# Project-Arda/bgls

Hardware: AMD Instinct MI355X
Metric: aggregate-verify signer-pairs/sec (higher is better)
Workload: dtype u32; 1 GPU; altbn128 VerifyAggregateSignature, one 1048576-signer batch, keys+msgs resident in HBM; curve=altbn128, signers=1048576, signers_per_gpu=1048576, in_flight=8

## Files before the change

bgls_amd/csrc/fp.hpp:

```cpp
#pragma once
#include <stdint.h>
#include "constants_gen.hpp"

#if defined(__HIPCC__)
#include <hip/hip_runtime.h>
#define BGLS_HD __host__ __device__ __forceinline__
#define BGLS_FN __host__ __device__ __noinline__
#else
#define BGLS_HD inline __attribute__((always_inline))
#define BGLS_FN __attribute__((noinline))
#endif

namespace bgls {

typedef uint32_t u32;
typedef uint64_t u64;
typedef int32_t i32;
typedef int64_t i64;

BGLS_HD u32 addc(u32 a, u32 b, u32& c) {
  u32 co;
  u32 r = __builtin_addc(a, b, c, &co);
  c = co;
  return r;
// ... 393 lines not shown
BGLS_FN Fp<C> fp_inv_ds(const Fp<C>& a) {
  constexpr int L = C::L;
  constexpr int NW = (32 * L + 29) / 30 + ((32 * L) % 30 == 0 ? 1 : 0);
  constexpr i32 M30 = (i32)((1u << 30) - 1u);
  static_assert(30 * NW >= 32 * L + 2, "limbs hold (-2p, 2p)");
  auto limb = [](const u32* w, int i) -> i32 {
    const int bit = 30 * i, q = bit >> 5, sh = bit & 31;
    if (q >= L) return 0;
    u64 x = w[q];
    if (q + 1 < L) x |= (u64)w[q + 1] << 32;
    return (i32)((u32)(x >> sh) & (u32)M30);
  };
  i32 f[NW], g[NW], d[NW], e[NW], m[NW];
#pragma unroll
  for (int i = 0; i < NW; ++i) {
    m[i] = limb(C::P, i);
    f[i] = m[i];
    g[i] = limb(a.v, i);
    d[i] = 0;
    e[i] = i == 0 ? 1 : 0;
  }
  u32 minv = C::P[0];
  minv *= 2u - C::P[0] * minv;
  minv *= 2u - C::P[0] * minv;
  minv *= 2u - C::P[0] * minv;
  minv *= 2u - C::P[0] * minv;
  minv *= 2u - C::P[0] * minv;
  i32 zeta = -1;
  for (int batch = 0; batch < 64; ++batch) {
    i32 u = 1, v = 0, q = 0, r = 1;
    {
      u32 fl = (u32)f[0] | ((u32)f[1] << 30), gl = (u32)g[0] | ((u32)g[1] << 30);
#pragma unroll
      for (int i = 0; i < 30; ++i) {
        i32 c1 = zeta >> 31;
        const i32 c2 = -(i32)(gl & 1u);
        const u32 x = (fl ^ (u32)c1) - (u32)c1;
        const i32 y = (u ^ c1) - c1, z = (v ^ c1) - c1;
        gl += x & (u32)c2;
        q += y & c2;
        r += z & c2;
        c1 &= c2;
        zeta = (zeta ^ c1) - 1;
        fl += gl & (u32)c1;
        u += q & c1;
        v += r & c1;
        gl >>= 1;
        u = (i32)((u32)u << 1);
        v = (i32)((u32)v << 1);
      }
    }
    {
      const i32 sd = d[NW - 1] >> 31, se = e[NW - 1] >> 31;
      i32 md = (u & sd) + (v & se), me = (q & sd) + (r & se);
      i64 cd = (i64)u * d[0] + (i64)v * e[0], ce = (i64)q * d[0] + (i64)r * e[0];
      md -= (i32)((minv * (u32)cd + (u32)md) & (u32)M30);
      me -= (i32)((minv * (u32)ce + (u32)me) & (u32)M30);
      cd += (i64)m[0] * md;
      ce += (i64)m[0] * me;
      cd >>= 30;
      ce >>= 30;
#pragma unroll
      for (int i = 1; i < NW; ++i) {
        cd += (i64)u * d[i] + (i64)v * e[i] + (i64)m[i] * md;
        ce += (i64)q * d[i] + (i64)r * e[i] + (i64)m[i] * me;
        d[i - 1] = (i32)cd & M30;
        e[i - 1] = (i32)ce & M30;
        cd >>= 30;
        ce >>= 30;
      }
      d[NW - 1] = (i32)cd;
      e[NW - 1] = (i32)ce;
    }
    u32 gnz;
    {
      i64 cf = (i64)u * f[0] + (i64)v * g[0], cg = (i64)q * f[0] + (i64)r * g[0];
      cf >>= 30;
      cg >>= 30;
      gnz = 0;
#pragma unroll
      for (int i = 1; i < NW; ++i) {
        cf += (i64)u * f[i] + (i64)v * g[i];
        cg += (i64)q * f[i] + (i64)r * g[i];
        f[i - 1] = (i32)cf & M30;
        g[i - 1] = (i32)cg & M30;
        gnz |= (u32)g[i - 1];
        cf >>= 30;
        cg >>= 30;
      }
      f[NW - 1] = (i32)cf;
      g[NW - 1] = (i32)cg;
      gnz |= (u32)g[NW - 1];
    }
#if defined(__HIP_DEVICE_COMPILE__)
    if (__ballot(gnz != 0) == 0ull) break;
#else
    if (gnz == 0) break;
#endif
  }
  u32 fone = (u32)f[0] ^ 1u, fmone = (u32)(f[0] ^ M30);
#pragma unroll
  for (int i = 1; i < NW; ++i) { fone |= (u32)f[i]; fmone |= (u32)(f[i] ^ (i == NW - 1 ? -1 : M30)); }
  if (fone != 0 && fmone != 0) return fp_zero<C>();
  const i32 sf = fone == 0 ? 0 : -1;
  i64 c = 0;
  u32 w[L + 1];
  {
    u64 acc = 0;
    int have = 0, wi = 0;
    i64 carry = 0;
#pragma unroll
    for (int i = 0; i < NW; ++i) {
      carry += (i64)((d[i] ^ sf) - sf) + 2 * (i64)m[i];
      const u32 lo = (u32)carry & (u32)M30;
      carry >>= 30;
      acc |= (u64)lo << have;
      have += 30;
      if (have >= 32) {
        if (wi <= L) w[wi] = (u32)acc;
        ++wi;
        acc >>= 32;
        have -= 32;
      }
    }
    acc |= (u64)(u32)carry << have;
    while (wi <= L) { w[wi++] = (u32)acc; acc >>= 32; }
    (void)c;
  }
  Fp<C> rr;
#pragma unroll
  for (int j = 0; j < L; ++j) rr.v[j] = w[j];
  u32 top = w[L];
#pragma unroll
  for (int k = 0; k < 4; ++k) {
    u32 bw = 0;
    u32 t[L];
#pragma unroll
    for (int j = 0; j < L; ++j) t[j] = subb(rr.v[j], C::P[j], bw);
    const bool ge = top != 0 || bw == 0;
    if (ge) {
#pragma unroll
      for (int j = 0; j < L; ++j) rr.v[j] = t[j];
      top -= bw;
    }
  }
  const Fp<C> r2 = fp_load<C>(C::R2);
  return fp_mul_inl<C>(fp_mul_inl<C>(rr, r2), r2);
}
template <class C>
BGLS_HD Fp<C> fp_inv(const Fp<C>& a) {
  return fp_inv_ds<C>(a);
}

template <int L, int LC>
BGLS_HD void fp_jacobi_phase(u32 (&a)[L], u32 (&n)[L], u32& t, bool& done) {
  for (int guard = 0; guard < 64 * L + 64; ++guard) {
    if (!done) {
      const u32 low = a[0];
      const u32 sft = low ? (u32)__builtin_ctz(low) : 31u;
#pragma unroll
      for (int j = 0; j < LC - 1; ++j) a[j] = (u32)((((u64)a[j + 1] << 32) | a[j]) >> sft);
      a[LC - 1] >>= sft;
      const u32 n8 = n[0] & 7u;
      t ^= (sft & 1u) & (u32)(n8 == 3u || n8 == 5u);
      const bool odd = (a[0] & 1u) != 0;
      u32 d[LC], e[LC];
      u32 bw = 0, bw2 = 0;
#pragma unroll
      for (int j = 0; j < LC; ++j) d[j] = subb(a[j], n[j], bw);
#pragma unroll
      for (int j = 0; j < LC; ++j) e[j] = subb(n[j], a[j], bw2);
      const bool lt = bw != 0;
      const bool swp = odd && lt;
      t ^= (u32)(swp && (a[0] & 3u) == 3u && (n[0] & 3u) == 3u);
      u32 z = 0;
#pragma unroll
      for (int j = 0; j < LC; ++j) {
        const u32 na = odd ? (lt ? e[j] : d[j]) : a[j];
        n[j] = swp ? a[j] : n[j];
        a[j] = na;
        z |= na;
      }
      if (z == 0) done = true;
    }
    bool again = !done, shrink = false;
    if constexpr (LC > 2) shrink = !done && ((a[LC - 1] | a[LC - 2] | n[LC - 1] | n[LC - 2]) != 0);
#if defined(__HIP_DEVICE_COMPILE__)
    again = __ballot(again) != 0;
    if constexpr (LC > 2) shrink = __ballot(shrink) != 0;
#endif
    if (!again) return;
    if constexpr (LC > 2) {
      if (!shrink) return;
    }
  }
}
template <int L, int LC>
BGLS_HD void fp_jacobi_phases(u32 (&a)[L], u32 (&n)[L], u32& t, bool& done) {
  fp_jacobi_phase<L, LC>(a, n, t, done);
  if constexpr (LC > 2) fp_jacobi_phases<L, LC - 2>(a, n, t, done);
}
template <class C>
BGLS_FN int fp_jacobi(const Fp<C>& x) {
  constexpr int L = C::L;
  static_assert(L % 2 == 0, "limb pairs");
  u32 a[L], n[L];
  u32 nz = 0;
#pragma unroll
  for (int j = 0; j < L; ++j) {
    a[j] = x.v[j];
    n[j] = C::P[j];
    nz |= a[j];
  }
  u32 t = 0;
  bool done = nz == 0;
  fp_jacobi_phases<L, L>(a, n, t, done);
  if (nz == 0) return 0;
  u32 one = n[0] ^ 1u;
#pragma unroll
  for (int j = 1; j < L; ++j) one |= n[j];
  if (one != 0) return 0;
  return t ? -1 : 1;
}

template <class C>
BGLS_HD Fp<C> fp_sqrt_candidate(const Fp<C>& a) {
  return fp_pow_w4<C, C::L>(a, C::EXP_SQRT);
}

template <class C>
BGLS_HD Fp<C> fp_from_be(const uint8_t* b) {
  Fp<C> r;
#pragma unroll
  for (int j = 0; j < C::L; ++j) {
    const uint8_t* q = b + 4 * (C::L - 1 - j);
    r.v[j] = ((u32)q[0] << 24) | ((u32)q[1] << 16) | ((u32)q[2] << 8) | (u32)q[3];
  }
  return r;
}

template <class C>
BGLS_HD void fp_to_be(uint8_t* b, const Fp<C>& a) {
#pragma unroll
  for (int j = 0; j < C::L; ++j) {
    uint8_t* q = b + 4 * (C::L - 1 - j);
    q[0] = (uint8_t)(a.v[j] >> 24);
    q[1] = (uint8_t)(a.v[j] >> 16);
    q[2] = (uint8_t)(a.v[j] >> 8);
    q[3] = (uint8_t)(a.v[j]);
  }
}

}
```

bgls_amd/csrc/h2c.hpp:

```cpp
#pragma once
#include "curve.hpp"
#include "hashes.hpp"

namespace bgls {

inline BGLS_FN bool bn_h2c_try(const uint8_t* msg, size_t len, u32 counter, Fp<BN254>& x, Fp<BN254>& r) {
  typedef BN254 C;
  ByteSrc src;
  src.msg = msg;
  src.len = len;
  src.pre[0] = (uint8_t)counter;
  src.npre = 1;
  src.nsuf = 0;
  u32 d[8];
  keccak256_legacy(src, d);
  Fp<C> h;
#pragma unroll
  for (int j = 0; j < 8; ++j) h.v[j] = d[7 - j];
  x = fp_to_mont<C>(h);
  Fp<C> y2 = fp_add<C>(fp_mul<C>(fp_sqr<C>(x), x), fp_load<C>(C::B));
  r = fp_sqrt_candidate<C>(y2);
  return fp_eq<C>(fp_sqr<C>(r), y2);
}

inline BGLS_FN bool bn_h2c_test(const uint8_t* msg, size_t len, u32 counter, Fp<BN254>& x, Fp<BN254>& y2) {
  typedef BN254 C;
  ByteSrc src;
  src.msg = msg;
  src.len = len;
  src.pre[0] = (uint8_t)counter;
  src.npre = 1;
  src.nsuf = 0;
  u32 d[8];
  keccak256_legacy(src, d);
  Fp<C> h;
#pragma unroll
  for (int j = 0; j < 8; ++j) h.v[j] = d[7 - j];
  x = fp_to_mont<C>(h);
  y2 = fp_add<C>(fp_mul<C>(fp_sqr<C>(x), x), fp_load<C>(C::B));
  return fp_jacobi<C>(y2) >= 0;
}

inline BGLS_FN u32 bn_h2c_sign(const uint8_t* msg, size_t len) {
  ByteSrc src;
  src.msg = msg;
  src.len = len;
  src.pre[0] = 0xFF;
  src.npre = 1;
  src.nsuf = 0;
  u32 d[8];
  keccak256_legacy(src, d);
  return d[7] & 1u;
}

inline BGLS_FN bool bn_hash_to_g1(const uint8_t* msg, size_t len, Aff<F1<BN254>>& out) {
  typedef BN254 C;
  for (u32 c = 0; c < 256; ++c) {
    Fp<C> x, r;
    if (bn_h2c_try(msg, len, c, x, r)) {
      if (bn_h2c_sign(msg, len)) r = fp_neg<C>(r);
      out.x = x;
      out.y = r;
      out.inf = false;
      return true;
    }
  }
  return false;
}

template <class C>
BGLS_HD bool fp_plain_parity(const Fp<C>& a) {
  Fp<C> d;
  u32 bw = 0;
#pragma unroll
  for (int j = 0; j < C::L; ++j) d.v[j] = subb(C::P[j], a.v[j], bw);
  u32 b2 = 0;
#pragma unroll
  for (int j = 0; j < C::L; ++j) (void)subb(d.v[j], a.v[j], b2);
  return b2 != 0;
}

inline BGLS_FN void bls_h2c_digest(const uint8_t* msg, size_t len, int k, u32 (&d)[16]) {
  ByteSrc src;
  src.msg = msg;
  src.len = len;
  src.npre = 0;
  src.pre[0] = 0;
  src.suf[0] = 'G';
  src.suf[1] = '1';
  src.suf[2] = '_';
  src.suf[3] = (uint8_t)('0' + k);
  src.nsuf = 4;
  blake2b512(src, d);
}
inline BGLS_FN Fp<BLS381> bls_h2c_t(const uint8_t* msg, size_t len, int k, Fp<BLS381>& t_mont) {
  typedef BLS381 C;
  u32 d[16];
  bls_h2c_digest(msg, len, k, d);
  Fp<C> lo, hi = fp_zero<C>();
#pragma unroll
  for (int j = 0; j < 12; ++j) lo.v[j] = d[15 - j];
#pragma unroll
  for (int j = 0; j < 4; ++j) hi.v[j] = d[3 - j];
  t_mont = fp_add<C>(fp_mul<C>(lo, fp_load<C>(C::R2)), fp_mul<C>(hi, fp_load<C>(C::R3)));
  return fp_from_mont<C>(t_mont);
}

inline BGLS_FN Aff<F1<BLS381>> bls_sw_encode(const Fp<BLS381>& t_mont, bool t_parity) {
  typedef BLS381 C;
  const Fp<C> one = fp_one<C>();
  const Fp<C> b = fp_load<C>(C::B);
  Fp<C> t2 = fp_sqr<C>(t_mont);
  Fp<C> u = fp_add<C>(fp_add<C>(t2, one), b);
  Fp<C> v = fp_mul3<C>(t2);
  Fp<C> I = fp_inv<C>(fp_mul<C>(u, v));
  Fp<C> inv_u = fp_mul<C>(I, v);
  Fp<C> w = fp_mul<C>(fp_mul<C>(fp_load<C>(C::SQRT_M3), t_mont), inv_u);
  Fp<C> x = fp_sub<C>(fp_load<C>(C::Z_SW), fp_mul<C>(t_mont, w));
  Fp<C> y;
  bool found = false;
  for (int i = 0; i < 3 && !found; ++i) {
    if (i == 1) x = fp_sub<C>(fp_neg<C>(x), one);
    if (i == 2) x = fp_sub<C>(one, fp_mul<C>(fp_mul<C>(fp_sqr<C>(u), u), I));
    Fp<C> g = fp_add<C>(fp_mul<C>(fp_sqr<C>(x), x), b);
    y = fp_sqrt_candidate<C>(g);
    found = (i == 2) || fp_eq<C>(fp_sqr<C>(y), g);
  }
  if (fp_plain_parity<C>(fp_from_mont<C>(y)) != t_parity) y = fp_neg<C>(y);
  return {x, y, false};
}

enum : u32 { H2C_INF = 0, H2C_PLUS_G1 = 1, H2C_MINUS_G1 = 2, H2C_SW = 3, H2C_PENDING = 4 };

struct BlsSwPrep {
  Fp<BLS381> x0, x2;
};
inline BGLS_FN BlsSwPrep bls_sw_prep(const Fp<BLS381>& t_mont) {
  typedef BLS381 C;
  const Fp<C> one = fp_one<C>();
  Fp<C> t2 = fp_sqr<C>(t_mont);
  Fp<C> u = fp_add<C>(fp_add<C>(t2, one), fp_load<C>(C::B));
  Fp<C> v = fp_mul3<C>(t2);
  Fp<C> I = fp_inv<C>(fp_mul<C>(u, v));
  Fp<C> w = fp_mul<C>(fp_mul<C>(fp_load<C>(C::SQRT_M3), t_mont), fp_mul<C>(I, v));
  BlsSwPrep r;
  r.x0 = fp_sub<C>(fp_load<C>(C::Z_SW), fp_mul<C>(t_mont, w));
  r.x2 = fp_sub<C>(one, fp_mul<C>(fp_mul<C>(fp_sqr<C>(u), u), I));
  return r;
}
inline BGLS_FN bool bls_sw_try(const Fp<BLS381>& x, Fp<BLS381>& y) {
  typedef BLS381 C;
  Fp<C> g = fp_add<C>(fp_mul<C>(fp_sqr<C>(x), x), fp_load<C>(C::B));
  y = fp_sqrt_candidate<C>(g);
  return fp_eq<C>(fp_sqr<C>(y), g);
}

template <class F>
BGLS_FN Jac<F> jac_mul_jac(const Jac<F>& p, const u32* k, int nbits) {
  Jac<F> r = jac_inf<F>();
  for (int i = nbits - 1; i >= 0; --i) {
    r = jac_dbl<F>(r);
    if ((k[i >> 5] >> (i & 31)) & 1u) r = jac_add<F>(r, p);
  }
  return r;
}

inline BGLS_FN Jac<F1<BLS381>> bls_hash_to_g1_jac(const uint8_t* msg, size_t len) {
  typedef BLS381 C;
  typedef F1<C> F;
  Jac<F> sw_sum = jac_inf<F>();
  Jac<F> special = jac_inf<F>();
  const Aff<F> g1 = {fp_load<C>(C::G1X), fp_load<C>(C::G1Y), false};
  for (int k = 0; k < 2; ++k) {
    Fp<C> tm;
    Fp<C> t = bls_h2c_t(msg, len, k, tm);
    if (fp_is_zero<C>(t)) continue;
    if (fp_eq<C>(t, fp_load<C>(C::FT_ROOT1))) {
      special = jac_add_aff<F>(special, g1);
    } else if (fp_eq<C>(t, fp_load<C>(C::FT_ROOT2))) {
      special = jac_add_aff<F>(special, aff_neg<F>(g1));
    } else {
      sw_sum = jac_add_aff<F>(sw_sum, bls_sw_encode(tm, fp_plain_parity<C>(t)));
    }
  }
  Jac<F> r = jac_mul_jac<F>(sw_sum, C::COFACTOR, C::COFACTOR_BITS);
  return jac_add<F>(r, special);
}

inline BGLS_FN Aff<F1<BLS381>> bls_hash_to_g1(const uint8_t* msg, size_t len) {
  return jac_to_aff<F1<BLS381>>(bls_hash_to_g1_jac(msg, len));
}

}
```

bgls_amd/csrc/hashes.hpp:

```cpp
#pragma once
#include "fp.hpp"

namespace bgls {

struct ByteSrc {
  const uint8_t* msg;
  size_t len;
  uint8_t pre[1];
  int npre;
  uint8_t suf[4];
  int nsuf;
  BGLS_HD size_t total() const { return (size_t)npre + len + (size_t)nsuf; }
  BGLS_HD u32 at(size_t pos) const {
    if (pos < (size_t)npre) return pre[0];
    pos -= npre;
    if (pos < len) return msg[pos];
    pos -= len;
    return suf[pos & 3];
  }
  BGLS_HD u64 le64(size_t pos, size_t total) const {
    if (pos >= (size_t)npre && pos + 8 <= (size_t)npre + len) {
      u64 w;
      __builtin_memcpy(&w, msg + (pos - (size_t)npre), 8);
      return w;
    }
    u64 w = 0;
#pragma unroll
    for (int b = 0; b < 8; ++b) {
      const size_t q = pos + b;
      const u32 byte = q < total ? at(q) : 0u;
      w |= (u64)byte << (8 * b);
    }
    return w;
  }
};

BGLS_HD u64 rotl64(u64 x, int n) { return (x << n) | (x >> (64 - n)); }
BGLS_HD u64 rotr64(u64 x, int n) { return (x >> n) | (x << (64 - n)); }

#if defined(__HIP_DEVICE_COMPILE__)
#define BGLS_TABLE __device__ __constant__ const
#else
#define BGLS_TABLE static const
#endif

BGLS_TABLE u64 KECCAK_RC[24] = {
    0x0000000000000001ull, 0x0000000000008082ull, 0x800000000000808Aull, 0x8000000080008000ull,
    0x000000000000808Bull, 0x0000000080000001ull, 0x8000000080008081ull, 0x8000000000008009ull,
    0x000000000000008Aull, 0x0000000000000088ull, 0x0000000080008009ull, 0x000000008000000Aull,
    0x000000008000808Bull, 0x800000000000008Bull, 0x8000000000008089ull, 0x8000000000008003ull,
    0x8000000000008002ull, 0x8000000000000080ull, 0x000000000000800Aull, 0x800000008000000Aull,
    0x8000000080008081ull, 0x8000000000008080ull, 0x0000000080000001ull, 0x8000000080008008ull};

BGLS_HD void keccak_f1600(u64 (&st)[25]) {
  constexpr int rotc[24] = {1, 3, 6, 10, 15, 21, 28, 36, 45, 55, 2, 14, 27, 41, 56, 8, 25, 43, 62, 18, 39, 61, 20, 44};
  constexpr int piln[24] = {10, 7, 11, 17, 18, 3, 5, 16, 8, 21, 24, 4, 15, 23, 19, 13, 12, 2, 20, 14, 22, 9, 6, 1};
  for (int round = 0; round < 24; ++round) {
    u64 bc[5];
#pragma unroll
    for (int i = 0; i < 5; ++i) bc[i] = st[i] ^ st[i + 5] ^ st[i + 10] ^ st[i + 15] ^ st[i + 20];
#pragma unroll
    for (int i = 0; i < 5; ++i) {
      u64 t = bc[(i + 4) % 5] ^ rotl64(bc[(i + 1) % 5], 1);
#pragma unroll
      for (int j = 0; j < 25; j += 5) st[j + i] ^= t;
    }
    u64 t = st[1];
#pragma unroll
    for (int i = 0; i < 24; ++i) {
      int j = piln[i];
      u64 b0 = st[j];
      st[j] = rotl64(t, rotc[i]);
      t = b0;
    }
#pragma unroll
    for (int j = 0; j < 25; j += 5) {
#pragma unroll
      for (int i = 0; i < 5; ++i) bc[i] = st[j + i];
#pragma unroll
      for (int i = 0; i < 5; ++i) st[j + i] ^= (~bc[(i + 1) % 5]) & bc[(i + 2) % 5];
    }
    st[0] ^= KECCAK_RC[round];
  }
}

inline BGLS_FN void keccak256_legacy(const ByteSrc& src, u32 (&out_be)[8]) {
  constexpr size_t RATE = 136;
  u64 st[25];
#pragma unroll
  for (int i = 0; i < 25; ++i) st[i] = 0;
  const size_t total = src.total();
  const size_t nblk = total / RATE + 1;
  for (size_t blk = 0; blk < nblk; ++blk) {
    const bool last = (blk + 1 == nblk);
#pragma unroll
    for (int i = 0; i < 17; ++i) {
      const size_t pos = blk * RATE + 8 * i;
      u64 w = src.le64(pos, total);
      if (total >= pos && total < pos + 8) w |= (u64)0x01u << (8 * (total - pos));
      if (last && i == 16) w ^= (u64)0x80u << 56;
      st[i] ^= w;
    }
    keccak_f1600(st);
  }
#pragma unroll
  for (int i = 0; i < 4; ++i) {
    u32 lo = (u32)st[i], hi = (u32)(st[i] >> 32);
    out_be[2 * i] = __builtin_bswap32(lo);
    out_be[2 * i + 1] = __builtin_bswap32(hi);
  }
}

BGLS_TABLE u64 BLAKE2B_IV[8] = {0x6a09e667f3bcc908ull, 0xbb67ae8584caa73bull, 0x3c6ef372fe94f82bull,
                                0xa54ff53a5f1d36f1ull, 0x510e527fade682d1ull, 0x9b05688c2b3e6c1full,
                                0x1f83d9abfb41bd6bull, 0x5be0cd19137e2179ull};
BGLS_TABLE uint8_t BLAKE2B_SIGMA[12][16] = {
    {0, 1, 2, 3, 4, 5, 6, 7, 8, 9, 10, 11, 12, 13, 14, 15}, {14, 10, 4, 8, 9, 15, 13, 6, 1, 12, 0, 2, 11, 7, 5, 3},
    {11, 8, 12, 0, 5, 2, 15, 13, 10, 14, 3, 6, 7, 1, 9, 4}, {7, 9, 3, 1, 13, 12, 11, 14, 2, 6, 5, 10, 4, 0, 15, 8},
    {9, 0, 5, 7, 2, 4, 10, 15, 14, 1, 11, 12, 6, 8, 3, 13}, {2, 12, 6, 10, 0, 11, 8, 3, 4, 13, 7, 5, 15, 14, 1, 9},
    {12, 5, 1, 15, 14, 13, 4, 10, 0, 7, 6, 3, 9, 2, 8, 11}, {13, 11, 7, 14, 12, 1, 3, 9, 5, 0, 15, 4, 8, 6, 2, 10},
    {6, 15, 14, 9, 11, 3, 0, 8, 12, 2, 13, 7, 1, 4, 10, 5}, {10, 2, 8, 4, 7, 6, 1, 5, 15, 11, 9, 14, 3, 12, 13, 0},
    {0, 1, 2, 3, 4, 5, 6, 7, 8, 9, 10, 11, 12, 13, 14, 15}, {14, 10, 4, 8, 9, 15, 13, 6, 1, 12, 0, 2, 11, 7, 5, 3}};

BGLS_HD void blake2b_g(u64 (&v)[16], int a, int b, int c, int d, u64 x, u64 y) {
  v[a] = v[a] + v[b] + x;
  v[d] = rotr64(v[d] ^ v[a], 32);
  v[c] = v[c] + v[d];
  v[b] = rotr64(v[b] ^ v[c], 24);
  v[a] = v[a] + v[b] + y;
  v[d] = rotr64(v[d] ^ v[a], 16);
  v[c] = v[c] + v[d];
  v[b] = rotr64(v[b] ^ v[c], 63);
}

BGLS_HD void blake2b_compress(u64 (&h)[8], const u64 (&m)[16], u64 t, bool last) {
  u64 v[16];
#pragma unroll
  for (int i = 0; i < 8; ++i) {
    v[i] = h[i];
    v[i + 8] = BLAKE2B_IV[i];
  }
  v[12] ^= t;
  if (last) v[14] = ~v[14];
  for (int r = 0; r < 12; ++r) {
    const uint8_t* s = BLAKE2B_SIGMA[r];
    blake2b_g(v, 0, 4, 8, 12, m[s[0]], m[s[1]]);
    blake2b_g(v, 1, 5, 9, 13, m[s[2]], m[s[3]]);
    blake2b_g(v, 2, 6, 10, 14, m[s[4]], m[s[5]]);
    blake2b_g(v, 3, 7, 11, 15, m[s[6]], m[s[7]]);
    blake2b_g(v, 0, 5, 10, 15, m[s[8]], m[s[9]]);
    blake2b_g(v, 1, 6, 11, 12, m[s[10]], m[s[11]]);
    blake2b_g(v, 2, 7, 8, 13, m[s[12]], m[s[13]]);
    blake2b_g(v, 3, 4, 9, 14, m[s[14]], m[s[15]]);
  }
#pragma unroll
  for (int i = 0; i < 8; ++i) h[i] ^= v[i] ^ v[i + 8];
}

inline BGLS_FN void blake2b512(const ByteSrc& src, u32 (&out_be)[16]) {
  u64 h[8];
#pragma unroll
  for (int i = 0; i < 8; ++i) h[i] = BLAKE2B_IV[i];
  h[0] ^= 0x01010040ull;
  const size_t total = src.total();
  const size_t nblk = total == 0 ? 1 : (total + 127) / 128;
  for (size_t blk = 0; blk < nblk; ++blk) {
    u64 m[16];
    for (int i = 0; i < 16; ++i) m[i] = src.le64(blk * 128 + 8 * (size_t)i, total);
    const bool last = (blk + 1 == nblk);
    blake2b_compress(h, m, last ? (u64)total : (u64)(blk + 1) * 128, last);
  }
#pragma unroll
  for (int i = 0; i < 8; ++i) {
    u32 lo = (u32)h[i], hi = (u32)(h[i] >> 32);
    out_be[2 * i] = __builtin_bswap32(lo);
    out_be[2 * i + 1] = __builtin_bswap32(hi);
  }
}

BGLS_HD void blake2xb_root_init(u64 (&h)[8], u32 xof_len) {
#pragma unroll
  for (int i = 0; i < 8; ++i) h[i] = BLAKE2B_IV[i];
  h[0] ^= 0x01010040ull;
  h[1] ^= (u64)xof_len << 32;
}
inline BGLS_FN void blake2xb_node(const u64 (&root)[8], u32 i, u32 xof_len, u32 take, u64 (&out)[8]) {
#pragma unroll
  for (int k = 0; k < 8; ++k) out[k] = BLAKE2B_IV[k];
  out[0] ^= (u64)take | (64ull << 32);
  out[1] ^= (u64)i | ((u64)xof_len << 32);
  out[2] ^= 64ull << 8;
  u64 m[16];
#pragma unroll
  for (int k = 0; k < 8; ++k) {
    m[k] = root[k];
    m[k + 8] = 0;
  }
  blake2b_compress(out, m, 64, true);
}

}
```

bgls_amd/csrc/k_hash.hip:

```cpp
#include <stdlib.h>
#include "dev_common.hpp"
#include "h2c.hpp"
#include "launch.hpp"
#include "rx_pow.hpp"
#include "rx_jac1.hpp"
#include "h2c_x.hpp"

using namespace bgls;

__device__ __forceinline__ uint64_t msg_hash64(const uint8_t* p, size_t n, uint64_t seed) {
  uint64_t h = 0xcbf29ce484222325ull ^ seed;
  for (size_t i = 0; i < n; ++i) {
    h ^= p[i];
    h *= 0x100000001b3ull;
  }
  h ^= h >> 29;
  h *= 0xbf58476d1ce4e5b9ull;
  h ^= h >> 32;
  return h;
}

__global__ void k_dup_check(MsgView mv, size_t n, uint32_t* table, uint32_t mask, uint32_t* flags, uint32_t bucket, uint32_t n_buckets, uint32_t max_probe,
                            uint64_t seed) {
  size_t i = blockIdx.x * (size_t)blockDim.x + threadIdx.x;
// ... 24 lines not shown
  }
  atomicOr(flags, FLAG_DUP);
}

__device__ __forceinline__ uint32_t inst_of(const uint64_t* inst_off, uint32_t n_inst, size_t i) {
  uint32_t lo = 0, hi = n_inst;
  while (hi - lo > 1) {
    const uint32_t mid = (lo + hi) >> 1;
    if (inst_off[mid] <= i) lo = mid;
    else hi = mid;
  }
  return lo;
}
__global__ void k_dup_check_seg(MsgView mv, size_t n, const uint64_t* inst_off, uint32_t n_inst, uint32_t* table, uint32_t mask, uint32_t* inst_flags,
                                uint64_t seed) {
  size_t i = blockIdx.x * (size_t)blockDim.x + threadIdx.x;
  if (i >= n) return;
  const uint32_t b = inst_of(inst_off, n_inst, i);
  const uint8_t* m = mv.ptr(i);
  const size_t len = mv.size(i);
  uint32_t slot = (uint32_t)msg_hash64(m, len, seed ^ (0x9e3779b97f4a7c15ull * (b + 1ull))) & mask;
  for (;;) {
    uint32_t prev = atomicCAS(&table[slot], 0u, (uint32_t)i + 1u);
    if (prev == 0u) return;
    size_t j = prev - 1u;
    if (inst_of(inst_off, n_inst, j) == b && mv.size(j) == len) {
      const uint8_t* o = mv.ptr(j);
      bool same = true;
      for (size_t k = 0; k < len; ++k)
        if (o[k] != m[k]) {
          same = false;
          break;
        }
      if (same) {
        atomicOr(&inst_flags[b], FLAG_DUP);
        return;
      }
    }
    slot = (slot + 1u) & mask;
  }
}

template <int LPM>
__global__ void __launch_bounds__(64, 3) k_h2c_bn_round(MsgView mv, size_t n, const uint32_t* list_in, const uint32_t* count_in,
                                                     uint32_t c0, uint32_t* list_out, uint32_t* count_out, int last,
                                                     Aff<F1<BN254>>* out, uint32_t* flags) {
  typedef BN254 C;
  const size_t count = count_in ? (size_t)*count_in : n;
  const size_t slots = (count * LPM + 63) / 64 * 64;
  const int lane = threadIdx.x;
  for (size_t slot = (size_t)blockIdx.x * 64 + lane; slot < slots; slot += (size_t)gridDim.x * 64) {
    const size_t item = slot / LPM;
    const uint32_t sub = (uint32_t)(slot % LPM);
    const uint32_t c = c0 + sub;
    const bool active = item < count && c < 256;
    size_t idx = 0;
    Fp<C> x, r;
    bool ok = false;
    if (item < count) idx = list_in ? list_in[item] : item;
    if (active) ok = bn_h2c_test(mv.ptr(idx), mv.size(idx), c, x, r);
    const unsigned long long ball = __ballot(ok);
    const int seg = (lane / LPM) * LPM;
    const unsigned long long segmask = LPM == 64 ? ball : ((ball >> seg) & ((1ull << (LPM & 63)) - 1ull));
    if (item < count) {
      if (segmask == 0) {
        if (sub == 0) {
          if (last) {
            atomicOr(flags, FLAG_HASH);
            out[idx] = {fp_zero<C>(), fp_zero<C>(), true};
          } else {
            list_out[atomicAdd(count_out, 1u)] = (uint32_t)idx;
          }
        }
      } else if (sub == (uint32_t)__builtin_ctzll(segmask)) {
        out[idx] = {x, r, false};
      }
    }
  }
}

constexpr int RXP_W = 3;
template <class C>
struct PowForm { typedef C type; };
template <>
struct PowForm<BN254> { typedef BN254W type; };
template <class C>
constexpr bool rxp_e0reg() { return C::CURVE_ID == 1; }
template <class C>
constexpr int rxp_lds_words() { return ((1 << (RXP_W - 1)) - (rxp_e0reg<C>() ? 1 : 0)) * PowForm<C>::type::RX_NL * 64; }
template <class C, bool M1>
__device__ __forceinline__ Fp<C> rx_sqrt_pow(const Fp<C>& a, i32* tab) {
  typedef typename PowForm<C>::type X;
  constexpr int N = X::RX_NL;
  const int lane = threadIdx.x & 63;
  auto ld = [&](int e, int i) { return tab[(e * N + i) * 64 + lane]; };
  auto st = [&](int e, int i, i32 v) { tab[(e * N + i) * 64 + lane] = v; };
  Fp<X> ax;
#pragma unroll
  for (int i = 0; i < C::L; ++i) ax.v[i] = a.v[i];
  const Sx<X, SX_T> r = sx_pow_sqrt<X, RXP_W, M1, rxp_e0reg<C>()>(ux_to_sx<X>(to_ux<X>(ax)), ld, st);
  Ux<X> u;
#pragma unroll
  for (int i = 0; i < N; ++i) u.v[i] = (u32)r.v[i];
  const Fp<X> rx = from_ux<X>(u);
  Fp<C> out;
#pragma unroll
  for (int i = 0; i < C::L; ++i) out.v[i] = rx.v[i];
  return out;
}

__global__ void __launch_bounds__(64, 3) k_h2c_bn_finish(MsgView mv, size_t n, Aff<F1<BN254>>* out) {
  typedef BN254 C;
  size_t i = blockIdx.x * (size_t)blockDim.x + threadIdx.x;
  if (i >= n) return;
  Aff<F1<C>> p = out[i];
  if (p.inf) return;
  __shared__ i32 tab[rxp_lds_words<C>()];
  Fp<C> r = rx_sqrt_pow<C, false>(p.y, tab);
  if (bn_h2c_sign(mv.ptr(i), mv.size(i))) r = fp_neg<C>(r);
  out[i].y = r;
}

#ifdef H2C_DBG
__device__ unsigned long long g_h2c_t[16];
#define H2C_T(k) do { if (blockIdx.x == 0 && threadIdx.x == 0) g_h2c_t[k] = clock64(); } while (0)
extern "C" int bgls_dbg_h2c_dump(unsigned long long* o) { return (int)hipMemcpyFromSymbol(o, HIP_SYMBOL(g_h2c_t), sizeof(g_h2c_t)); }
#else
#define H2C_T(k) do { } while (0)
#endif
__global__ void __launch_bounds__(64, 3) k_h2c_bn_wide(MsgView mv, size_t n, Aff<F1<BN254>>* out, uint32_t* flags) {
  typedef BN254 C;
  const int lane = threadIdx.x, sub = lane & 15, grp = lane >> 4;
  const size_t i = (size_t)blockIdx.x * 4 + grp;
  const bool live = i < n;
  const uint8_t* msg = mv.ptr(live ? i : 0);
  const size_t len = mv.size(live ? i : 0);
  __shared__ i32 tab[rxp_lds_words<C>()];
  Fp<C> x, y2;
  bool done = !live, mine = false;
  u32 sign = 0;
  u32 base = 0;
  bool first = true;
  for (;;) {
    const u32 c = first ? (sub == 15 ? 255u : (u32)sub) : base + (u32)sub;
    ByteSrc src;
    src.msg = msg; src.len = len; src.pre[0] = (uint8_t)c; src.npre = 1; src.nsuf = 0;
    u32 d[8];
    H2C_T(0);
    keccak256_legacy(src, d);
    H2C_T(1);
    Fp<C> h;
#pragma unroll
    for (int j = 0; j < 8; ++j) h.v[j] = d[7 - j];
    const Fp<C> xc = fp_to_mont<C>(h);
    const Fp<C> yc = fp_add<C>(fp_mul<C>(fp_sqr<C>(xc), xc), fp_load<C>(C::B));
    H2C_T(2);
    const Fp<C> rc = rx_sqrt_pow<C, false>(yc, tab);
    H2C_T(3);
    bool ok = fp_eq<C>(fp_sqr<C>(rc), yc) && c < 256u && !done;
    H2C_T(4);
    if (first) {
      sign = __shfl(d[7] & 1u, grp * 16 + 15);
      if (sub == 15) ok = false;
    }
    const unsigned long long ball = __ballot(ok);
    const u32 field = (u32)(ball >> (16 * grp)) & 0xFFFFu;
    if (!done && field) {
      mine = sub == (int)__builtin_ctz(field);
      done = true;
      if (mine) { x = xc; y2 = rc; }
    }
    base = first ? 15u : base + 16u;
    first = false;
    if (__ballot(!done) == 0ull || base >= 256u) break;
  }
  if (!done) {
    if (sub == 0) {
      atomicOr(flags, FLAG_HASH);
      out[i] = {fp_zero<C>(), fp_zero<C>(), true};
    }
    return;
  }
  H2C_T(5);
  if (mine) out[i] = {x, sign ? fp_neg<C>(y2) : y2, false};
  H2C_T(6);
}

__global__ void __launch_bounds__(64, 3) k_bls_sw_jacobi(MsgView mv, size_t n_items, Jac<F1<BLS381>>* pts, uint32_t* kinds) {
  typedef BLS381 C;
  constexpr int N = C::RX_NL;
  size_t item = blockIdx.x * (size_t)blockDim.x + threadIdx.x;
  if (item >= n_items) return;
  const size_t msg = item >> 1;
  u32 d[16];
  bls_h2c_digest(mv.ptr(msg), mv.size(msg), (int)(item & 1), d);
  __shared__ i32 tab[rxp_lds_words<C>()];
  const int lane = threadIdx.x & 63;
  auto ld = [&](int e, int i) { return tab[(e * N + i) * 64 + lane]; };
  auto st = [&](int e, int i, i32 w) { tab[(e * N + i) * 64 + lane] = w; };
  Jac<F1<C>> pt;
  const uint32_t kind = bls_sw_jac_x<RXP_W, rxp_e0reg<C>()>(d, pt, ld, st);
  kinds[item] = kind;
  if (kind == H2C_SW) pts[item] = pt;
}

template <bool RAW>
__global__ void __launch_bounds__(64) k_bls_combine(size_t n, const Jac<F1<BLS381>>* pts, const uint32_t* kinds, Aff<F1<BLS381>>* out) {
  typedef BLS381 C;
  typedef F1<C> F;
  size_t i = blockIdx.x * (size_t)blockDim.x + threadIdx.x;
  if (i >= n) return;
  Jac<F> sw = jac_inf<F>(), special = jac_inf<F>();
  const Aff<F> g1 = {fp_load<C>(RAW ? C::G1KX : C::G1X), fp_load<C>(RAW ? C::G1KY : C::G1Y), false};
  for (int k = 0; k < 2; ++k) {
    const uint32_t kind = kinds[2 * i + k];
    if (kind == H2C_SW) sw = jac_add<F>(sw, pts[2 * i + k]);
    else if (kind == H2C_PLUS_G1) special = jac_add_aff<F>(special, g1);
    else if (kind == H2C_MINUS_G1) special = jac_add_aff<F>(special, aff_neg<F>(g1));
  }
  if constexpr (RAW) {
    out[i] = jac_to_aff<F>(jac_add<F>(sw, special));
    return;
  }
  const Aff<F> S = jac_to_aff<F>(sw);
  const Aff<F> nS = aff_neg<F>(S);
  Jac<F> r = jac_inf<F>();
  for (int d = 0; d < C::COFACTOR_NAF_LEN; ++d) {
    r = jac_dbl<F>(r);
    const int dig = C::COFACTOR_NAF[d];
    if (dig != 0) r = jac_add_aff<F>(r, dig > 0 ? S : nS);
  }
  out[i] = jac_to_aff<F>(jac_add<F>(r, special));
}

__global__ void __launch_bounds__(64) k_bls_combine_x(size_t n, const Jac<F1<BLS381>>* pts, const uint32_t* kinds, Aff<F1<BLS381>>* out) {
  typedef BLS381 C;
  typedef F1<C> F;
  size_t i = blockIdx.x * (size_t)blockDim.x + threadIdx.x;
  if (i >= n) return;
  Jac<F> sw = jac_inf<F>(), special = jac_inf<F>();
  const Aff<F> g1 = {fp_load<C>(C::G1X), fp_load<C>(C::G1Y), false};
  for (int k = 0; k < 2; ++k) {
    const uint32_t kind = kinds[2 * i + k];
    if (kind == H2C_SW) sw = jac_add<F>(sw, pts[2 * i + k]);
    else if (kind == H2C_PLUS_G1) special = jac_add_aff<F>(special, g1);
    else if (kind == H2C_MINUS_G1) special = jac_add_aff<F>(special, aff_neg<F>(g1));
  }
  const Aff1<C> S = aff1_from_mont<C>(jac_to_aff<F>(sw));
  const Aff1<C> nS = aff1_neg<C>(S);
  Jac1<C> r = jac1_inf<C>();
#pragma unroll 1
  for (int d = 0; d < C::COFACTOR_NAF_LEN; ++d) {
    r = jac1_dbl<C>(r);
    const int dig = C::COFACTOR_NAF[d];
    if (dig != 0) r = jac1_madd<C>(r, dig > 0 ? S : nS);
  }
  out[i] = jac_to_aff<F>(jac_add<F>(jac1_to_mont<C>(r), special));
}

__global__ void __launch_bounds__(64) k_bls_combine_raw_x(size_t n, const Jac<F1<BLS381>>* pts, const uint32_t* kinds, Aff<F1<BLS381>>* out) {
  typedef BLS381 C;
  typedef F1<C> F;
  size_t i = blockIdx.x * (size_t)blockDim.x + threadIdx.x;
  if (i >= n) return;
  const Aff1<C> g1 = aff1_from_mont<C>(Aff<F>{fp_load<C>(C::G1KX), fp_load<C>(C::G1KY), false});
  Jac1<C> sw = jac1_inf<C>();
  for (int k = 0; k < 2; ++k) {
    const uint32_t kind = kinds[2 * i + k];
    if (kind == H2C_SW) {
      const Jac<F> q = pts[2 * i + k];
      Jac1<C> qx;
      qx.X = sx_as<SX_F, C>(sx_from_mont<C>(q.X));
      qx.Y = sx_as<SX_F, C>(sx_from_mont<C>(q.Y));
      qx.Z = sx_as<SX_F, C>(sx_from_mont<C>(q.Z));
      qx.inf = jac_is_inf<F>(q);
      sw = jac1_add<C>(sw, qx);
    } else if (kind == H2C_PLUS_G1) {
      sw = jac1_madd<C>(sw, g1);
    } else if (kind == H2C_MINUS_G1) {
      sw = jac1_madd<C>(sw, aff1_neg<C>(g1));
    }
  }
  if (sw.inf) {
    out[i] = {fp_zero<C>(), fp_zero<C>(), true};
    return;
  }
  const Sx<C, SX_T> zi = sx_from_mont<C>(fp_inv<C>(sx_to_mont<C>(sw.Z)));
  const Sx<C, SX_T> zi2 = s1_sqr<C>(zi);
  out[i] = {sx_to_mont<C>(s1_mul<C>(sw.X, zi2)), sx_to_mont<C>(s1_mul<C>(s1_mul<C>(sw.Y, zi2), zi)), false};
}

template <int KB>
__global__ void __launch_bounds__(64) k_bls_combine_raw_batched(size_t n, Jac<F1<BLS381>>* pts, const uint32_t* kinds, Aff<F1<BLS381>>* out) {
  typedef BLS381 C;
  typedef F1<C> F;
  const size_t i0 = (blockIdx.x * (size_t)blockDim.x + threadIdx.x) * KB;
  if (i0 >= n) return;
  const Aff<F> g1 = {fp_load<C>(C::G1KX), fp_load<C>(C::G1KY), false};
  Fp<C> pre[KB];
  Fp<C> run = fp_one<C>();
#pragma unroll 1
  for (int k = 0; k < KB; ++k) {
    const size_t i = i0 + k;
    if (i < n) {
      Jac<F> sw = jac_inf<F>();
      for (int h = 0; h < 2; ++h) {
        const uint32_t kind = kinds[2 * i + h];
        if (kind == H2C_SW) sw = jac_add<F>(sw, pts[2 * i + h]);
        else if (kind == H2C_PLUS_G1) sw = jac_add_aff<F>(sw, g1);
        else if (kind == H2C_MINUS_G1) sw = jac_add_aff<F>(sw, aff_neg<F>(g1));
      }
      pts[2 * i] = sw;
// ... 142 lines not shown
```

Baseline: 18.90 million signer-pairs/s.

## Inline hash-to-curve path, streamline Jacobi loop, add single-block Keccak absorb fast path

Rewrites the binary Jacobi symbol loop to track a nonzero word instead of a done flag, handle whole-zero-limb shifts separately, and use alignbit funnel shifts with simpler sign-update formulas. Adds a device fast path to Keccak that absorbs short single-block messages with a prefix byte through direct 8-byte loads. It also forces inlining of the field multiply and square helpers, the Jacobi routine and the hash-to-curve helpers, so the calls in the hashing kernel avoid noinline call overhead. In exchange, code size and register pressure may grow, and the fast path assumes unaligned 8-byte reads of messages are safe.

```diff
diff --git a/bgls_amd/csrc/fp.hpp b/bgls_amd/csrc/fp.hpp
--- a/bgls_amd/csrc/fp.hpp
+++ b/bgls_amd/csrc/fp.hpp
@@ -569,42 +569,48 @@
   return fp_inv_ds<C>(a);
 }
 
+BGLS_HD u32 funnel_shr(u32 hi, u32 lo, u32 s) {
+#if defined(__HIP_DEVICE_COMPILE__)
+  return __builtin_amdgcn_alignbit(hi, lo, s);
+#else
+  return (u32)((((u64)hi << 32) | lo) >> s);
+#endif
+}
 template <int L, int LC>
-BGLS_HD void fp_jacobi_phase(u32 (&a)[L], u32 (&n)[L], u32& t, bool& done) {
+BGLS_HD void fp_jacobi_phase(u32 (&a)[L], u32 (&n)[L], u32& t, u32& z) {
   for (int guard = 0; guard < 64 * L + 64; ++guard) {
-    if (!done) {
-      const u32 low = a[0];
-      const u32 sft = low ? (u32)__builtin_ctz(low) : 31u;
-#pragma unroll
-      for (int j = 0; j < LC - 1; ++j) a[j] = (u32)((((u64)a[j + 1] << 32) | a[j]) >> sft);
+    if (__builtin_expect(z != 0 && a[0] == 0, 0)) {
+#pragma unroll
+      for (int j = 0; j < LC - 1; ++j) a[j] = a[j + 1];
+      a[LC - 1] = 0;
+    } else if (z != 0) {
+      const u32 sft = (u32)__builtin_ctz(a[0]);
+#pragma unroll
+      for (int j = 0; j < LC - 1; ++j) a[j] = funnel_shr(a[j + 1], a[j], sft);
       a[LC - 1] >>= sft;
-      const u32 n8 = n[0] & 7u;
-      t ^= (sft & 1u) & (u32)(n8 == 3u || n8 == 5u);
-      const bool odd = (a[0] & 1u) != 0;
+      const u32 n0 = n[0];
+      t ^= sft & ((n0 ^ (n0 >> 1)) >> 1);
       u32 d[LC], e[LC];
       u32 bw = 0, bw2 = 0;
 #pragma unroll
-      for (int j = 0; j < LC; ++j) d[j] = subb(a[j], n[j], bw);
-#pragma unroll
-      for (int j = 0; j < LC; ++j) e[j] = subb(n[j], a[j], bw2);
-      const bool lt = bw != 0;
-      const bool swp = odd && lt;
-      t ^= (u32)(swp && (a[0] & 3u) == 3u && (n[0] & 3u) == 3u);
-      u32 z = 0;
-#pragma unroll
       for (int j = 0; j < LC; ++j) {
-        const u32 na = odd ? (lt ? e[j] : d[j]) : a[j];
-        n[j] = swp ? a[j] : n[j];
-        a[j] = na;
-        z |= na;
+        d[j] = subb(a[j], n[j], bw);
+        e[j] = subb(n[j], a[j], bw2);
       }
-      if (z == 0) done = true;
-    }
-    bool again = !done, shrink = false;
-    if constexpr (LC > 2) shrink = !done && ((a[LC - 1] | a[LC - 2] | n[LC - 1] | n[LC - 2]) != 0);
+      t ^= bw ? (a[0] & n0) >> 1 : 0u;
+      z = 0;
+#pragma unroll
+      for (int j = 0; j < LC; ++j) {
+        n[j] = bw ? a[j] : n[j];
+        a[j] = bw ? e[j] : d[j];
+        z |= a[j];
+      }
+    }
+    bool again = z != 0, shrink = false;
+    if constexpr (LC > 2) shrink = z != 0 && ((a[LC - 1] | a[LC - 2] | n[LC - 1] | n[LC - 2]) != 0);
 #if defined(__HIP_DEVICE_COMPILE__)
-    again = __ballot(again) != 0;
-    if constexpr (LC > 2) shrink = __ballot(shrink) != 0;
+    again = __builtin_amdgcn_ballot_w64(again) != 0ull;
+    if constexpr (LC > 2) shrink = __builtin_amdgcn_ballot_w64(shrink) != 0ull;
 #endif
     if (!again) return;
     if constexpr (LC > 2) {
@@ -613,12 +619,12 @@
   }
 }
 template <int L, int LC>
-BGLS_HD void fp_jacobi_phases(u32 (&a)[L], u32 (&n)[L], u32& t, bool& done) {
-  fp_jacobi_phase<L, LC>(a, n, t, done);
-  if constexpr (LC > 2) fp_jacobi_phases<L, LC - 2>(a, n, t, done);
-}
-template <class C>
-BGLS_FN int fp_jacobi(const Fp<C>& x) {
+BGLS_HD void fp_jacobi_phases(u32 (&a)[L], u32 (&n)[L], u32& t, u32& z) {
+  fp_jacobi_phase<L, LC>(a, n, t, z);
+  if constexpr (LC > 2) fp_jacobi_phases<L, LC - 2>(a, n, t, z);
+}
+template <class C>
+BGLS_HD int fp_jacobi_inl(const Fp<C>& x) {
   constexpr int L = C::L;
   static_assert(L % 2 == 0, "limb pairs");
   u32 a[L], n[L];
@@ -630,14 +636,18 @@
     nz |= a[j];
   }
   u32 t = 0;
-  bool done = nz == 0;
-  fp_jacobi_phases<L, L>(a, n, t, done);
+  u32 z = nz;
+  fp_jacobi_phases<L, L>(a, n, t, z);
   if (nz == 0) return 0;
   u32 one = n[0] ^ 1u;
 #pragma unroll
   for (int j = 1; j < L; ++j) one |= n[j];
   if (one != 0) return 0;
-  return t ? -1 : 1;
+  return (t & 1u) ? -1 : 1;
+}
+template <class C>
+BGLS_FN int fp_jacobi(const Fp<C>& x) {
+  return fp_jacobi_inl<C>(x);
 }
 
 template <class C>
diff --git a/bgls_amd/csrc/h2c.hpp b/bgls_amd/csrc/h2c.hpp
--- a/bgls_amd/csrc/h2c.hpp
+++ b/bgls_amd/csrc/h2c.hpp
@@ -23,7 +23,7 @@
   return fp_eq<C>(fp_sqr<C>(r), y2);
 }
 
-inline BGLS_FN bool bn_h2c_test(const uint8_t* msg, size_t len, u32 counter, Fp<BN254>& x, Fp<BN254>& y2) {
+BGLS_HD bool bn_h2c_test(const uint8_t* msg, size_t len, u32 counter, Fp<BN254>& x, Fp<BN254>& y2) {
   typedef BN254 C;
   ByteSrc src;
   src.msg = msg;
@@ -36,12 +36,12 @@
   Fp<C> h;
 #pragma unroll
   for (int j = 0; j < 8; ++j) h.v[j] = d[7 - j];
-  x = fp_to_mont<C>(h);
-  y2 = fp_add<C>(fp_mul<C>(fp_sqr<C>(x), x), fp_load<C>(C::B));
-  return fp_jacobi<C>(y2) >= 0;
+  x = fp_mul_inl<C>(h, fp_load<C>(C::R2));
+  y2 = fp_add<C>(fp_mul_inl<C>(fp_sqr_inl<C>(x), x), fp_load<C>(C::B));
+  return fp_jacobi_inl<C>(y2) >= 0;
 }
 
-inline BGLS_FN u32 bn_h2c_sign(const uint8_t* msg, size_t len) {
+BGLS_HD u32 bn_h2c_sign(const uint8_t* msg, size_t len) {
   ByteSrc src;
   src.msg = msg;
   src.len = len;
diff --git a/bgls_amd/csrc/hashes.hpp b/bgls_amd/csrc/hashes.hpp
--- a/bgls_amd/csrc/hashes.hpp
+++ b/bgls_amd/csrc/hashes.hpp
@@ -84,23 +84,55 @@
   }
 }
 
-inline BGLS_FN void keccak256_legacy(const ByteSrc& src, u32 (&out_be)[8]) {
+#if defined(__HIP_DEVICE_COMPILE__)
+#define BGLS_KECCAK_FN BGLS_HD
+#else
+#define BGLS_KECCAK_FN inline BGLS_FN
+#endif
+BGLS_KECCAK_FN void keccak256_legacy(const ByteSrc& src, u32 (&out_be)[8]) {
   constexpr size_t RATE = 136;
   u64 st[25];
 #pragma unroll
   for (int i = 0; i < 25; ++i) st[i] = 0;
   const size_t total = src.total();
   const size_t nblk = total / RATE + 1;
+  bool absorbed = false;
+#if defined(__HIP_DEVICE_COMPILE__)
+  const bool fast = src.npre == 1 && src.nsuf == 0 && src.len >= 8 && total < RATE;
+  if (__builtin_amdgcn_ballot_w64(!fast) == 0ull) {
+    const uint8_t* m = src.msg;
+    const u32 len = (u32)src.len;
+    u64 w0, wl;
+    __builtin_memcpy(&w0, m, 8);
+    __builtin_memcpy(&wl, m + (len - 8u), 8);
+    st[0] = (w0 << 8) | (u64)src.pre[0];
+    const u32 it = (len + 1u) >> 3;
+    const u32 k = (len + 1u) & 7u;
+    const u64 tail = ((wl >> 8) >> (8u * (7u - k))) | ((u64)0x01u << (8u * k));
+#pragma unroll
+    for (int i = 1; i < 17; ++i) {
+      u64 w = 0;
+      if (8u * (u32)i + 7u <= len) __builtin_memcpy(&w, m + (8 * i - 1), 8);
+      else if ((u32)i == it) w = tail;
+      st[i] = w;
+    }
+    st[16] ^= (u64)0x80u << 56;
+    absorbed = true;
+  }
+#endif
   for (size_t blk = 0; blk < nblk; ++blk) {
-    const bool last = (blk + 1 == nblk);
-#pragma unroll
-    for (int i = 0; i < 17; ++i) {
-      const size_t pos = blk * RATE + 8 * i;
-      u64 w = src.le64(pos, total);
-      if (total >= pos && total < pos + 8) w |= (u64)0x01u << (8 * (total - pos));
-      if (last && i == 16) w ^= (u64)0x80u << 56;
-      st[i] ^= w;
-    }
+    if (!absorbed) {
+      const bool last = (blk + 1 == nblk);
+#pragma unroll
+      for (int i = 0; i < 17; ++i) {
+        const size_t pos = blk * RATE + 8 * i;
+        u64 w = src.le64(pos, total);
+        if (total >= pos && total < pos + 8) w |= (u64)0x01u << (8 * (total - pos));
+        if (last && i == 16) w ^= (u64)0x80u << 56;
+        st[i] ^= w;
+      }
+    }
+    absorbed = false;
     keccak_f1600(st);
   }
 #pragma unroll
diff --git a/bgls_amd/csrc/k_hash.hip b/bgls_amd/csrc/k_hash.hip
--- a/bgls_amd/csrc/k_hash.hip
+++ b/bgls_amd/csrc/k_hash.hip
@@ -200,12 +200,12 @@
     Fp<C> h;
 #pragma unroll
     for (int j = 0; j < 8; ++j) h.v[j] = d[7 - j];
-    const Fp<C> xc = fp_to_mont<C>(h);
-    const Fp<C> yc = fp_add<C>(fp_mul<C>(fp_sqr<C>(xc), xc), fp_load<C>(C::B));
+    const Fp<C> xc = fp_mul_inl<C>(h, fp_load<C>(C::R2));
+    const Fp<C> yc = fp_add<C>(fp_mul_inl<C>(fp_sqr_inl<C>(xc), xc), fp_load<C>(C::B));
     H2C_T(2);
     const Fp<C> rc = rx_sqrt_pow<C, false>(yc, tab);
     H2C_T(3);
-    bool ok = fp_eq<C>(fp_sqr<C>(rc), yc) && c < 256u && !done;
+    bool ok = fp_eq<C>(fp_sqr_inl<C>(rc), yc) && c < 256u && !done;
     H2C_T(4);
     if (first) {
       sign = __shfl(d[7] & 1u, grp * 16 + 15);
```

Result: no change. 19.04 million signer-pairs/s (median of 6 runs) (+0.7%).
